# fusiyuan2010/CSC

Hardware: AMD Instinct MI355X
Metric: encode MB/s (10^6 input bytes / wall-clock) on enwik9 stand-in, -m3 -d64m; stream bit-exact vs reference (higher is better)
Workload: dtype u8/u32 (byte + 32-bit integer work; 12-bit probabilities, 64-bit range-coder low)

## Files before the change

csc_amd/csrc/csc_kernels_dp4.inc:

```

constexpr uint32_t kD4Rec = 256;
constexpr uint32_t kD4CandEnt = kD4Rec * 4;
constexpr uint32_t kD4RefEnt = 256;
constexpr uint32_t kD4Ent = kD4CandEnt + kD4RefEnt;
constexpr uint32_t kD4LA = 48;
constexpr uint32_t kD4Waves = 12;
DEV uint32_t d4_role(uint32_t w)
{
    constexpr uint32_t roles[12] = { 0, 6, 7, 1, 8, 5, 4, 2, 8, 8, 9, 3 };
    return w < 12 ? roles[w] : 8u;
}
constexpr uint32_t kD4Requested = 0xFFFFFFFFu;
#ifndef D4_IDLE_MUL
#define D4_IDLE_MUL 1
#endif
constexpr int kD4IdleSleep = 4 * D4_IDLE_MUL;
constexpr uint32_t kD4RefreshAt = 32;
constexpr uint32_t kD4MaxGood = 16;
constexpr uint32_t kD6Ring = 128;
constexpr uint32_t kD6MRing = 64;
constexpr uint32_t kD4MultiMax = 768;

struct Dp4X {
    uint32_t sb_seq, sb_ack, quit, abort;
// ... 1436 lines not shown
#ifdef CSCMI_TIMERS
                const uint32_t k_run0 = k;
#endif
                do {
#ifdef CSCMI_TIMERS_FINE
                    const unsigned long long tt0 = __builtin_readcyclecounter();
                    unsigned long long tt1 = 0;
#endif
                    pf_load();
                    d5_pad<D5_PAD_SPINE>();
                    const uint32_t st4 = (d5_bcast<D5F_BS>(LBL) >> 14) & 0xFCu;
                    const uint64_t tlr = *(volatile __attribute__((address_space(3))) uint64_t *)(b_tlr + (st4 << 4));
                    const uint32_t m32 = d5_bcast<D5F_M32>(LBL), tbu = d5_bcast<D5F_TBV>(LBL);
                    const uint32_t has1 = ((m32 & 3u) + 1u) >> 2;
                    const uint32_t p1f = tbu >> 16;
                    uint32_t E, cond0;
                    auto own = [&]() {
                        const uint32_t cl = tree + (tbu & 0xFFFFu);
                        const uint32_t k1m = (uint32_t)((int32_t)(p1f - cl) >> 31) & (0u - has1);
                        const uint32_t price = (p1f & k1m) | (cl & ~k1m);
                        const uint32_t eBS = k | (((st4 | (k1m & 2u)) & 0x3Fu) << 16);
                        const uint32_t tbE = ((uint32_t)(tlr >> 32) & k1m) | ((uint32_t)tlr & ~k1m);
                        E = (LBL >> shv) + ((price & mP) | c_left);
                        E = (eBS & mBS) | (E & ~mBS);
                        E = (k1m & 1u & mD) | (E & ~mD);
                        E = (tbE & mTBV) | (E & ~mTBV);
                        cond0 = (E & m_lsign) | ((v_lp - kD5Zone1) >> 31);
                    };
                    own();
                    const uint32_t want = winhi | k;
                    uint32_t late, wayout;
                    auto looks = [&]() {
                        late = (((uint32_t)prog - want) | ((uint32_t)(prog >> 32) - want)) >> 16;
                        const uint32_t g = (V.x ^ 1u) | (v_reach ^ j);
                        wayout = (V.w & D5V_OUT) | ((g - 1u) >> 31);
                    };
                    looks();
                    uint32_t LBLn, em;
                    auto merge = [&]() {
                        const uint32_t d = (T1 & mlow) - (T0 & mlow);
                        const uint32_t ds = (uint32_t)__builtin_amdgcn_mov_dpp((int)d, 0x55, 0xF, 0xF, false);
                        const uint32_t x = d != 0 ? d : ds;
                        const uint32_t t1 = d5_bcast<D5F_P>((uint32_t)((int32_t)x >> 31));
                        const uint32_t BEST = (T1 & t1) | (T0 & ~t1);
                        em = d5_bcast<D5F_P>((uint32_t)((int32_t)(E - BEST) >> 31));
                        LBLn = ((E & em) | (BEST & ~em)) | rfl;
                        asm volatile("" :: "v"(LBLn));
                    };
                    merge();
                    if (__builtin_expect(__ballot((late | wayout | cond0) != 0) != 0, 0)) {
                        if (__ballot(late != 0) != 0) {
                            uint32_t spins = 0;
                            for (;;) {
                                pf_load();
                                looks();
                                if (__ballot(late != 0) == 0) break;
                                if ((++spins & 0xFFFu) == 0 && (lds_vload(&X->abort) || spins > (kDpSpinLimit << 4))) {
                                    if (!lds_vload(&X->abort)) *(lds_vu32 *)&X->abort = 0x400D0000u | (k & 0xFFFFu);
                                    run = RUN_ABORT;
                                    break;
                                }
                            }
                            own();
                            merge();
#ifdef CSCMI_TIMERS_FINE
                            tt1 = __builtin_readcyclecounter();
#endif
                        }
                        if (run == RUN_ON && __ballot((wayout | cond0) != 0) != 0) {
                            const bool zone = __ballot(((v_lp - kD5Zone1) >> 31) != 0) != 0;
                            const bool out = __ballot(wayout != 0) != 0;
                            run = (zone || (out && D5DBG(8u))) ? RUN_GENERAL : out ? RUN_OUT : RUN_ASK;
                        }
                        if (run != RUN_ON) kstop = 0;
                    }
                    if (__builtin_expect(run == RUN_ON, 1)) {
                    LBL = LBLn;
                    *lds_at(st_a) = LBL;
                    k++;
                    *(lds_vu32 *)&X->lab_seq = k + 1u;
#ifdef CSCMI_TIMERS_FINE
                    if (tr_on && k <= 50) { unsigned long long *T = TR + (4 + k - 1) * 12; T[0] = tt0; T[1] = tt1; T[2] = __builtin_readcyclecounter(); T[8] = UNI(em) & 1u; }
#endif
                    st_a = (st_a & ~st_and) | ((st_a + st_inc) & st_and);
                    v_lp -= V.w & 0xFFFFu; v_reach = max(v_reach, j + V.x);
                    j = k - 1u;
                    pf_next();
                    }
                } while (k < kstop);
                vnext = j;
#ifdef CSCMI_TIMERS
                n_straight += k - k_run0;
#endif
                if (__builtin_expect(run != RUN_ON, 0)) {
                    const uint32_t wpos = sb0 + w0 + k;
                    if (run == RUN_ASK) {
                        const raw_vec4 e2 = *(lds_vvec4 *)&X->ent[(rdlane(LBL, D5F_I0) & 0xFFFFu) + vz];
                        uint32_t nm, nl;
                        mask_at(e2, wpos, nm, nl);
                        LBL = (nm & mM32) | (nl & c_left) | (LBL & ~(mM32 | c_left));
                        if (__ballot(nl == 0) == 0) continue;
#ifdef CSCMI_TIMERS
                        if (lane == 0) atomicAdd(&X->wtm[32], 1u);
#endif
                        leave = 1;
                    } else if (run == RUN_OUT) {
                        const uint32_t v0 = UNI(V.x), v1 = UNI(V.y), v2 = UNI(V.z), v3 = UNI(V.w);
                        v_lp -= v3 & 0xFFFFu;
                        if (j == 0 && (v3 & D5V_NONE)) { kind = DP_SEEN_EXIT; end = 0; }
                        else {
                            kind = (v0 == 1u) ? DP_EXIT_LIT : DP_EXIT_MATCH; end = j;
                            a0l = v0; a0code = v1; a0eid = v2 & 0xFFFFu; a0slot = v2 >> 16;
                        }
                        leave = 2;
                    } else if (run == RUN_ABORT) { err = 1; kind = DP_ABORT; leave = 2; }
                    else {
#ifdef CSCMI_TIMERS
                        if (lane == 0) atomicAdd(&X->wtm[35], 1u);
#endif
                        leave = 1;
                    }
                    break;
                }
            }
            vP = rdlane(LBL, D5F_P) | vz; vBS = rdlane(LBL, D5F_BS) | vz; vD = rdlane(LBL, D5F_D) | vz; vI0 = rdlane(LBL, D5F_I0) | vz; vI1 = rdlane(LBL, D5F_I1) | vz;
            if (leave == 2) break;
        }

        const uint32_t p = w0 + k, wpos = sb0 + p;
        *(lds_vu32 *)&X->m_pos = w0 + vnext; *(lds_vu32 *)&X->m_ids[0] = vI0; *(lds_vu32 *)&X->m_ids[1] = vI1;
        bool done = false;
        if (__builtin_expect(!done, 0)) {
#ifdef CSCMI_TIMERS
            const unsigned long long tg0 = __builtin_readcyclecounter();
            n_gen++;
#endif
            uint32_t cP = UNI(vP), cD = UNI(vD), cBS = UNI(vBS), cI0 = UNI(vI0), cI1 = UNI(vI1), lp_int = UNI(v_lp), reach = UNI(v_reach);
            const uint32_t state = (cBS >> 16) & 0x3Fu;
            bool out = false;
            uint32_t eP = kDpInf, eD = 0, eBS = 0;
            if (k < aplimit) {
                uint32_t rid_v = __builtin_amdgcn_perm(cI1, cI0, sel_rid);
                raw_vec4 en = *(lds_vvec4 *)&X->ent[rid_v];
                const uint32_t fwv = *(lds_vu32 *)&X->fwd[rid_v];
                const uint32_t tb = UNI(*(lds_vu32 *)&X->tab[state][8]);
                uint32_t tree = *(volatile __attribute__((address_space(3))) uint16_t *)&X->litp[lit_seq & 3u][p & (kD4Rec - 1)];
                {
                    const bool ask = (lane < 4) & (fwv == 0) & (wpos - en.y >= 64u) & (wpos - en.y < 0x80000000u);
                    if (__builtin_expect(__ballot(ask) != 0, 0)) rq_head = UNI(d4_ask(__ballot(ask), rid_v, wpos, rq_head));
                    const bool sw = (lane < 4) & (fwv != 0) & (fwv != kD4Requested);
                    if (__builtin_expect(__ballot(sw) != 0, 0)) {
                        lds_fence();
                        const uint32_t sm = 0u - (uint32_t)sw;
                        rid_v = ((fwv - 1u) & sm) | (rid_v & ~sm);
                        en = *(lds_vvec4 *)&X->ent[rid_v];
                        const uint32_t n0 = rdlane(rid_v, 0), n1 = rdlane(rid_v, 1), n2 = rdlane(rid_v, 2), n3 = rdlane(rid_v, 3);
                        cI0 = n0 | (n1 << 16); cI1 = n2 | (n3 << 16);
                    }
                }
                const uint32_t ex = UNI(en.x), ey = UNI(en.y), ez = UNI(en.z), ew = UNI(en.w);
                const uint32_t off = wpos - ey;
                const uint64_t m = (((uint64_t)ew << 32) | ez) >> (off & 63u);
                const uint32_t room = 64u - (off & 63u);
                uint32_t rl0 = umin((~m) ? (uint32_t)__builtin_ctzll(~m) : 64u, room);
                if (__builtin_expect(off >= 64u || rl0 >= room || (ey < ex && ex <= wpos), 0)) rl0 = UNI(d4_rep_direct(true, wpos, ex, size - p));
                const uint32_t has1 = rl0 >= 2u ? 1u : 0u;
                if (__builtin_expect(p >= lit_ok, 0)) {
                    lit_ok = UNI(d4_wait_lit(p, lit_seq & 0x3FFFFu));
                    if (!lit_ok) { err = 1; kind = DP_ABORT; out = true; }
                    tree = *(volatile __attribute__((address_space(3))) uint16_t *)&X->litp[lit_seq & 3u][p & (kD4Rec - 1)];
                }
                const uint32_t litf = tb & 0xFFFFu, p1f = tb >> 16;
                uint32_t c1 = UNI(tree) + litf, k1 = 0;
                if (has1 && p1f < c1) { c1 = p1f; k1 = 1; }
                eP = cP + c1; eD = k1; eBS = k | (((state * 4u + (k1 ? 2u : 0u)) & 0x3Fu) << 16);
            }
            if (__builtin_expect(lp_int < 192u && !have_new, 0)) { d6_wait_match_trees(); d4_len_price_rebuild(X->lenp_new); have_new = 1; }
            for (uint32_t pass = 0; pass < 2 && !out; pass++) {
                if (pass == 1 && !(lp_int < kD5Zone2 && k < aplimit)) break;
                const uint32_t vneed = k + pass;
                if (!d5_wait_edges(X, winhi, vneed, k, vz)) { err = 1; kind = DP_ABORT; out = true; break; }
                lds_fence();
                for (; vnext < vneed; vnext++) {
                    const uint32_t j = vnext;
                    const raw_vec4 V = *(lds_vvec4 *)&X->ver[j & 15u];
                    const uint32_t v0 = UNI(V.x), v1 = UNI(V.y), v2 = UNI(V.z), v3 = UNI(V.w);
                    const uint32_t nt = v3 & 0xFFFFu;
                    if (j == 0 && (v3 & D5V_NONE)) { kind = DP_SEEN_EXIT; end = 0; out = true; break; }
                    if (v3 & D5V_PRICED) {
                        if (lp_int < nt) { lp_int = 4096u - (nt - lp_int - 1u); refreshed = 1; }
                        else lp_int -= nt;
                    }
                    const bool exit_lit = v0 == 1 && reach == j;
                    const bool exit_match = v0 >= good || (v0 > 1 && v0 + j >= aplimit);
                    if (exit_lit || exit_match) {
                        kind = exit_lit ? DP_EXIT_LIT : DP_EXIT_MATCH; end = j;
                        a0l = v0; a0code = v1; a0eid = v2 & 0xFFFFu; a0slot = v2 >> 16;
                        out = true;
                        break;
                    }
                    reach = max(reach, j + v0);
                }
            }
            if (!out && k == aplimit) { kind = DP_EXIT_LIMIT; end = k; out = true; }
            if (!out) {
                const uint32_t t = k + 1u;
                uint32_t bP = kDpInf, bD = 0, bBS = 0, bI0 = 0, bI1 = 0;
                if (k >= 1) {
                    const raw_vec4 A = *(lds_vvec4 *)&X->tent[t & 1u][t & 15u][0];
                    bP = UNI(A.x); bBS = UNI(A.y); bD = UNI(A.z); bI0 = UNI(A.w); bI1 = UNI(*(lds_vu32 *)&X->tent[t & 1u][t & 15u][4]);
                }
                if (k >= 2) {
                    const raw_vec4 B = *(lds_vvec4 *)&X->tent[k & 1u][t & 15u][0];
                    const uint32_t qP = UNI(B.x), qBS = UNI(B.y), qD = UNI(B.z), qI0 = UNI(B.w), qI1 = UNI(*(lds_vu32 *)&X->tent[k & 1u][t & 15u][4]);
                    if (qP < bP || (qP == bP && (qBS & 0xFFFFu) < (bBS & 0xFFFFu))) { bP = qP; bD = qD; bBS = qBS; bI0 = qI0; bI1 = qI1; }
                }
                if (eP < bP) { bP = eP; bD = eD; bBS = eBS; bI0 = cI0; bI1 = cI1; }
                cP = bP; cD = bD; cBS = bBS; cI0 = bI0; cI1 = bI1;
                k++;
                raw_vec4 lb;
                lb.x = cP; lb.y = cBS | (refreshed << 31) | (lp_int < kD5Zone2 ? (lp_int + 1u) << 24 : 0u); lb.z = cI0; lb.w = cI1;
                *(lds_vvec4 *)&X->lab[k & 15u] = lb;
                L->fin2[k * 2u] = cD; L->fin2[k * 2u + 1u] = cBS;
#ifdef CSCMI_TIMERS
                if (k < 64) { X->dbgq[k][0] = cP; X->dbgq[k][5] = eP; X->dbgq[k][6] = 2; X->dbgq[k][7] = lp_int; }
#endif
                lds_fence();
                *(lds_vu32 *)&X->lab_seq = k + 1u;
            }
            vP = cP | vz; vD = cD | vz; vBS = cBS | vz; vI0 = cI0 | vz; vI1 = cI1 | vz; v_lp = lp_int | vz; v_reach = reach | vz;
            fI0 = cI0; fI1 = cI1;
            if (!out) pf_label();
#ifdef CSCMI_TIMERS
            t_gen += __builtin_readcyclecounter() - tg0;
#endif
            if (out) break;
        }
    }
#ifdef CSCMI_TIMERS
    const unsigned long long tse = __builtin_readcyclecounter();
    if (lane == 0) { atomicAdd(&X->wtm[13], (uint32_t)(tse - ts0) >> 4); atomicAdd(&X->wtm[14], n_straight); atomicAdd(&X->wtm[15], 1u);
        atomicAdd(&X->wtm[24], (uint32_t)(ts0 - tsp) >> 4); atomicAdd(&X->wtm[25], (uint32_t)t_first >> 4); atomicAdd(&X->wtm[26], (uint32_t)t_poll >> 4);
        atomicAdd(&X->wtm[27], (uint32_t)t_gen >> 4); atomicAdd(&X->wtm[28], n_gen); atomicAdd(&X->wtm[29], (uint32_t)(tse - t_last) >> 4); }
#endif
    lds_fence();
    *(lds_vu32 *)&X->lab_seq = kD5Stop;
    if (refreshed) { if (lane < 32) L->len_price[lane] = X->lenp_new[lane]; lds_fence(); }
    uint32_t f0 = kind == DP_EXIT_LIMIT ? fI0 : UNI(X->lab[end & 15u].z);
    uint32_t f1 = kind == DP_EXIT_LIMIT ? fI1 : UNI(X->lab[end & 15u].w);
    d5_forward_ids(X, lane, sel_rid, f0, f1);
    *(lds_vu32 *)&X->m_pos = w0 + end; *(lds_vu32 *)&X->m_ids[0] = f0; *(lds_vu32 *)&X->m_ids[1] = f1;
    {
        raw_vec4 o0, o1, o2;
        o0.x = kind; o0.y = end; o0.z = a0l; o0.w = a0code; o1.x = a0eid; o1.y = a0slot; o1.z = f0; o1.w = f1;
        o2.x = v_lp; o2.y = lit_seq; o2.z = rq_head; o2.w = err;
        *(lds_vvec4 *)&X->o_kind = o0; *(lds_vvec4 *)&X->o_a0eid = o1; *(lds_vvec4 *)&X->o_lp_int = o2;
    }
    lds_fence();
#ifdef CSCMI_TIMERS
    if (lane == 0) atomicAdd(&X->wtm[30], (uint32_t)(__builtin_readcyclecounter() - tse) >> 4);
#endif
}

DEV void d4_request(Sc &c, Dp4X *X, uint32_t id, uint32_t base, uint32_t &rq_head)
{
    if (rq_head - lds_vload(&X->rq_tail) >= 16u) return;
    X->rq[rq_head & 15u][0] = id;
    X->rq[rq_head & 15u][1] = base;
    X->fwd[id] = kD4Requested;
    rq_head++;
    lds_fence();
    lds_vstore(&X->rq_head, rq_head);
}

DEV bool d4_rebase_reps(Sc &c, Dp4X *X, uint32_t base, uint32_t &rq_head, bool wait)
{
    for (uint32_t r = 0; r < 4; r++) {
        const uint32_t id = lds_vload(&X->rid[r]);
        const uint32_t f = lds_vload(&X->fwd[id]);
        if (f == 0) {
            uint32_t spins = 0;
            while (rq_head - lds_vload(&X->rq_tail) >= 16u) if (!d4_spin(c, X, spins, 3)) return false;
            d4_request(c, X, id, base, rq_head);
        }
    }
    if (!wait) return true;
    for (uint32_t r = 0; r < 4; r++) {
        uint32_t id = lds_vload(&X->rid[r]);
        uint32_t spins = 0, f;
        while ((f = lds_vload(&X->fwd[id])) == kD4Requested) if (!d4_spin(c, X, spins, 4)) return false;
        if (f) { lds_fence(); X->rid[r] = f - 1; }
    }
    return true;
}


struct D6Cur { uint32_t lt_head, lt_seen, mt_head, mt_seen; };
DEV bool d6_join(Sc &c, Dp4X *X, D6Cur &q, bool lit_only = false);
DEV bool d6_room(Sc &c, Dp4X *X, uint32_t need, D6Cur &q)
{
    if (__builtin_expect(c.q_room < need, 0)) {
#ifdef CSCMI_TIMERS
        const uint64_t t0 = __builtin_readcyclecounter();
#endif
        if (!d6_join(c, X, q)) return false;
#ifdef CSCMI_TIMERS
        const uint64_t t1 = __builtin_readcyclecounter();
#endif
        q_publish(c);
        c.q_room = kCoderQ - 64u - q_wait_room(c, 64u + need);
#ifdef CSCMI_TIMERS
        if (c.lane == 0) { atomicAdd(&X->wtm[40], 1u); atomicAdd(&X->wtm[41], (uint32_t)(t1 - t0) >> 4); atomicAdd(&X->wtm[42], (uint32_t)(__builtin_readcyclecounter() - t1) >> 4); atomicAdd(&X->wtm[46], c.q_room >> 4); }
#endif
    }
    return true;
}
DEV bool d6_literal(Sc &c, Dp4X *X, uint32_t sym, D6Cur &q)
{
    if (__builtin_expect(q.lt_head - q.lt_seen >= kD6Ring - 8u, 0)) {
        uint32_t spins = 0;
        while (q.lt_head - (q.lt_seen = lds_vload(&X->lt_done)) >= kD6Ring - 8u) if (!d4_spin(c, X, spins, 12)) return false;
    }
    const uint32_t fidx = P_STATE + c.state * 3;
    const uint32_t pold = c.L->P[fidx];
    c.L->P[fidx] = p_update(0, pold);
    c.Q->e[c.q_head & (kCoderQ - 1)] = 0x80000000u | pold;
    *(lds_vu32 *)&X->lt_rec[q.lt_head & (kD6Ring - 1)] = c.ctx | (sym << 8) | (c.q_head << 16);
    q.lt_head++;
    *(lds_vu32 *)&X->lt_pub = q.lt_head;
    c.q_head += 9; c.q_room -= 9;
    c.state = (c.state * 4) & 0x3F;
    c.ctx = sym;
    c.st_lit++;
    return true;
}
DEV void d6_flags(Sc &c, uint32_t nf, uint32_t idx, uint32_t bit)
{
    const bool on = c.lane < nf;
    const uint32_t i = on ? idx : kPDumpE;
    const uint32_t p = c.L->P[i];
    c.L->P[i] = p + (uint32_t)((int32_t)((bit ? 0xFFFu : 31u) - p) >> 5);
    c.Q->e[(c.q_head + (on ? c.lane : 63u)) & (kCoderQ - 1)] = 0x80000000u | (bit << 12) | p;
    c.q_head += nf; c.q_room -= nf;
}
DEV uint32_t d6_len_slots(uint32_t len) { return len < 8 ? 4u : len < 16 ? 5u : 9u; }
DEV bool d6_tree_record(Sc &c, Dp4X *X, uint32_t w0, uint32_t w1, uint32_t nslots, D6Cur &q)
{
    if (__builtin_expect(q.mt_head - q.mt_seen >= kD6MRing, 0)) {
        uint32_t spins = 0;
        while (q.mt_head - (q.mt_seen = lds_vload(&X->mt_done)) >= kD6MRing) if (!d4_spin(c, X, spins, 14)) return false;
    }
    *(lds_vu32 *)&X->mt_rec[q.mt_head & (kD6MRing - 1)][0] = w0 | (c.q_head << 16);
    *(lds_vu32 *)&X->mt_rec[q.mt_head & (kD6MRing - 1)][1] = w1;
    q.mt_head++;
    *(lds_vu32 *)&X->mt_pub = q.mt_head;
    c.q_head += nslots; c.q_room -= nslots;
    return true;
}
DEV bool d6_match(Sc &c, Dp4X *X, uint32_t dist, uint32_t len, D6Cur &q)
{
    d6_flags(c, 2, P_STATE + c.state * 3 + c.lane, 1u);
    const uint32_t sbits = len == 0 ? 3u : len <= 2 ? 4u : 5u;
    const uint32_t slot = dist_slot(dist), extra_bits = slot > 2 ? slot - 2 : 0;
    const uint32_t ndir = extra_bits > 4 ? (extra_bits - 4 > 16 ? 2u : 1u) : 0u;
    if (!d6_tree_record(c, X, 0u | (len << 1), dist, d6_len_slots(len) + sbits + ndir + (extra_bits ? 4u : 0u), q)) return false;
    c.state = (c.state * 4 + 1) & 0x3F;
    c.st_match++;
    return true;
}
DEV bool d6_rep_match(Sc &c, Dp4X *X, uint32_t rep_idx, uint32_t len, D6Cur &q)
{
    const uint32_t s3 = c.state * 3, k = c.lane;
    const uint32_t idx = k < 3 ? P_STATE + s3 + k : P_REPDIST + s3 - 1u + (k == 3 ? 1u : 2u | (rep_idx >> 1));
    const uint32_t bit = k < 3 ? (0x5u >> k) & 1u : (rep_idx >> ((4u - k) & 1u)) & 1u;
    d6_flags(c, 5, idx, bit);
    if (!d6_tree_record(c, X, 1u | (len << 1), 0u, d6_len_slots(len), q)) return false;
    c.state = (c.state * 4 + 3) & 0x3F;
    c.st_match++;
    return true;
}
DEV void d6_rep0len1(Sc &c)
{
    d6_flags(c, 3, P_STATE + c.state * 3 + c.lane, c.lane == 0 ? 1u : 0u);
    c.ctx = 0;
    c.state = (c.state * 4 + 2) & 0x3F;
    c.st_match++;
}
DEV bool d6_encode_nonlit(Sc &c, Dp4X *X, uint32_t ulen, uint32_t udist, D6Cur &q)
{
    EncLds *L = c.L;
    if (udist <= 4) {
        if (ulen == 1 && udist == 1) d6_rep0len1(c);
        else {
            if (!d6_rep_match(c, X, udist - 1, ulen - 2, q)) return false;
            uint32_t d = UNI(L->rep[udist - 1]);
            for (uint32_t k = udist - 1; k > 0; k--) L->rep[k] = UNI(L->rep[k - 1]);
            L->rep[0] = d;
        }
    } else {
        if (!d6_match(c, X, udist - 5, ulen - 2, q)) return false;
        uint32_t r0 = UNI(L->rep[0]), r1 = UNI(L->rep[1]), r2 = UNI(L->rep[2]);
        L->rep[3] = r2; L->rep[2] = r1; L->rep[1] = r0; L->rep[0] = udist - 4;
    }
    return true;
}
DEV uint32_t d6_chunk_shape(uint32_t nd, uint32_t ql, bool on)
{
    const uint32_t len = ql & 0xFFFFu;
    const uint32_t kind = nd == 0 ? 0u : nd > 4 ? 1u : (nd == 1 && len == 1) ? 2u : 3u;
    const uint32_t l2 = len - 2u, dist = nd - 5u;
    const uint32_t sbits = l2 == 0 ? 3u : l2 <= 2 ? 4u : 5u;
    const uint32_t slot = dist_slot(dist), extra_bits = slot > 2 ? slot - 2 : 0;
    const uint32_t ndir = extra_bits > 4 ? (extra_bits - 4 > 16 ? 2u : 1u) : 0u;
    const uint32_t nf = kind == 0 ? 1u : kind == 1 ? 2u : kind == 2 ? 3u : 5u;
    const uint32_t tree = kind == 0 ? 8u : kind == 2 ? 0u : d6_len_slots(l2) + (kind == 1 ? sbits + ndir + (extra_bits ? 4u : 0u) : 0u);
    return on ? kind | (nf << 2) | ((nf + tree) << 8) : 0u;
}
DEV void d6_chunk_flag(bool act, uint32_t idx, uint32_t bit, uint32_t qslot, uint64_t same)
{
    const uint64_t am = __ballot(act);
    if (am == 0) return;
    const uint32_t lane = threadIdx.x & 63u;
    same &= am;
    const uint64_t below = same & ((1ull << lane) - 1ull), above = (same >> lane) >> 1;
    const uint32_t rank = (uint32_t)__builtin_popcountll(below);
    const uint32_t prev = below ? 63u - (uint32_t)__builtin_clzll(below) : lane;
    uint32_t pold = 0;
    if (act) pold = g_lds4.base.P[idx];
    uint32_t pnew = p_update(bit, pold);
    for (uint32_t d = 1; __ballot(act && rank >= d) != 0; d++) {
        const uint32_t v = (uint32_t)__builtin_amdgcn_ds_bpermute((int)(prev * 4u), (int)pnew);
        if (act && rank == d) { pold = v; pnew = p_update(bit, pold); }
    }
    if (act && above == 0) g_lds4.base.P[idx] = pnew;
    if (act) g_lds4.q.e[qslot & (kCoderQ - 1)] = 0x80000000u | (bit << 12) | pold;
}
__device__ __noinline__ uint32_t d6_chunk_lanes(uint32_t nd, uint32_t ql, uint32_t shape, uint32_t qpos, uint32_t n_, uint32_t state0_, uint32_t ctx0_, uint32_t lt_head_, uint32_t mt_head_)
{
    Dp4X *X = &g_lds4.x;
    const uint32_t lane = threadIdx.x & 63u;
    const uint32_t n = UNI(n_), state0 = UNI(state0_), ctx0 = UNI(ctx0_), lt_head = UNI(lt_head_), mt_head = UNI(mt_head_);
    const bool on = lane < n;
    const uint32_t kind = shape & 3u, nf = (shape >> 2) & 7u;
    const uint32_t len = ql & 0xFFFFu, last = ql >> 16;
    const uint64_t b0 = __ballot(on && (kind & 1u)), b1 = __ballot(on && (kind & 2u));
    const uint64_t h0 = (b0 << 3) | ((state0 & 1u) << 2) | (((state0 >> 2) & 1u) << 1) | ((state0 >> 4) & 1u);
    const uint64_t h1 = (b1 << 3) | (((state0 >> 1) & 1u) << 2) | (((state0 >> 3) & 1u) << 1) | ((state0 >> 5) & 1u);
    const uint32_t a = (uint32_t)(lane >= 3 ? b0 >> (lane - 3u) : h0 >> lane) & 7u, b = (uint32_t)(lane >= 3 ? b1 >> (lane - 3u) : h1 >> lane) & 7u;
    const uint32_t state = ((a >> 2) & 1u) | (((b >> 2) & 1u) << 1) | (((a >> 1) & 1u) << 2) | (((b >> 1) & 1u) << 3) | ((a & 1u) << 4) | ((b & 1u) << 5);
    const uint32_t before = (uint32_t)__shfl_up((int)last, 1);
    const uint32_t ctx = lane == 0 ? ctx0 : before;
    const bool is_lit = on && kind == 0, has_tree = on && (kind & 1u);
    const uint64_t lm = __ballot(is_lit), tm = __ballot(has_tree);
    if (is_lit) {
        const uint32_t r = __builtin_amdgcn_mbcnt_hi((uint32_t)(lm >> 32), __builtin_amdgcn_mbcnt_lo((uint32_t)lm, 0u));
        *(lds_vu32 *)&X->lt_rec[(lt_head + r) & (kD6Ring - 1)] = ctx | (last << 8) | (qpos << 16);
    }
    if (lm) lds_vstore(&X->lt_pub, lt_head + (uint32_t)__builtin_popcountll(lm));
    if (has_tree) {
        const uint32_t r = __builtin_amdgcn_mbcnt_hi((uint32_t)(tm >> 32), __builtin_amdgcn_mbcnt_lo((uint32_t)tm, 0u));
        *(lds_vu32 *)&X->mt_rec[(mt_head + r) & (kD6MRing - 1)][0] = (kind == 3 ? 1u : 0u) | ((len - 2u) << 1) | ((qpos + nf) << 16);
        *(lds_vu32 *)&X->mt_rec[(mt_head + r) & (kD6MRing - 1)][1] = kind == 1 ? nd - 5u : 0u;
    }
    if (tm) lds_vstore(&X->mt_pub, mt_head + (uint32_t)__builtin_popcountll(tm));
    uint64_t same = 0;
    for (uint64_t rem = __ballot(on); rem;) {
        const uint32_t sv = rdlane(state, (uint32_t)__builtin_ctzll(rem));
        const uint64_t mm = __ballot(on && state == sv);
        same = state == sv ? mm : same;
        rem &= ~mm;
    }
    const uint32_t s3 = state * 3u, rep_hi = ((nd - 1u) >> 1) & 1u;
    const bool is_rep = on && kind == 3;
    d6_chunk_flag(on, P_STATE + s3, kind != 0 ? 1u : 0u, qpos, same);
    d6_chunk_flag(on && kind != 0, P_STATE + s3 + 1u, kind == 1 ? 1u : 0u, qpos + 1u, same);
    d6_chunk_flag(on && kind >= 2, P_STATE + s3 + 2u, kind == 3 ? 1u : 0u, qpos + 2u, same);
    d6_chunk_flag(is_rep, P_REPDIST + s3, rep_hi, qpos + 3u, same);
    const uint64_t hi = __ballot(is_rep && rep_hi);
    d6_chunk_flag(is_rep, P_REPDIST + s3 + 1u + rep_hi, (nd - 1u) & 1u, qpos + 4u, same & (rep_hi ? hi : ~hi));
    return rdlane(((state * 4u + kind) & 0x3Fu) | (last << 8), n - 1u);
}
DEV bool d6_join(Sc &c, Dp4X *X, D6Cur &q, bool lit_only)
{
    uint32_t spins = 0;
    if (q.lt_seen != q.lt_head) {
        while ((q.lt_seen = lds_vload(&X->lt_done)) != q.lt_head) if (!d4_spin(c, X, spins, 13)) return false;
        dp_fence();
    }
    if (!lit_only && q.mt_seen != q.mt_head) {
        while ((q.mt_seen = lds_vload(&X->mt_done)) != q.mt_head) if (!d4_spin(c, X, spins, 15)) return false;
        lds_fence();
    }
    return true;
}
DEV void d6_trees(Sc &c)
{
    Dp4X *X = d4x(c);
    uint32_t done = 0, mdone = 0;
  for (;;) {
    uint32_t pub, mpub, idle = 0;
    for (;;) {
        pub = lds_vload(&X->lt_pub); mpub = lds_vload(&X->mt_pub);
        if (pub != done || mpub != mdone) break;
        if (lds_vload(&X->quit) || lds_vload(&X->abort)) return;
        if (idle < 48u) { idle++; __builtin_amdgcn_s_sleep(1 * D4_IDLE_MUL); }
        else __builtin_amdgcn_s_sleep(6 * D4_IDLE_MUL);
    }
    if (pub == done) {
        const uint32_t w0 = lds_vload(&X->mt_rec[mdone & (kD6MRing - 1)][0]), dist = lds_vload(&X->mt_rec[mdone & (kD6MRing - 1)][1]);
        const uint32_t len = (w0 >> 1) & 0xFFu, qpos = w0 >> 16;
        Decisions d; d.idx = 0; d.bit = 0; d.n = 0;
        dec_matchlen_1(c, d, len);
        uint32_t n_head = d.n, extra_bits = 0, extra_len = 0;
        if ((w0 & 1u) == 0) {
            uint32_t pdist_pos, sbits;
            if (len == 0) { pdist_pos = 0; sbits = 3; }
            else if (len <= 2) { pdist_pos = 16 * (len - 1) + 8; sbits = 4; }
            else if (len <= 5) { pdist_pos = 32 * (len - 3) + 8 + 16 * 2; sbits = 5; }
            else { pdist_pos = 32 * 3 + 8 + 16 * 2; sbits = 5; }
            const uint32_t slot = dist_slot(dist);
            extra_bits = slot > 2 ? slot - 2 : 0;
            dec_tree(c, d, P_DIST + pdist_pos, slot, sbits);
            n_head = d.n;
            if (extra_bits) {
                extra_len = dist - (1u << extra_bits) - 1;
                dec_tree(c, d, P_DIST_EXTRA + (extra_bits - 1) * 16, __brev(extra_len & 0x0Fu) >> 28, 4);
            }
        }
        const uint32_t pold = dec_apply(c, d);
        uint32_t ndir = 0;
        if (extra_bits > 4) {
            const uint32_t v = extra_len >> 4, l = extra_bits - 4;
            if (l <= 16) { g_lds4.q.e[(qpos + n_head) & (kCoderQ - 1)] = 0x40000000u | (l << 16) | (v & 0xFFFFu); ndir = 1; }
            else { g_lds4.q.e[(qpos + n_head) & (kCoderQ - 1)] = 0x40000000u | ((l - 16) << 16) | ((v >> 16) & 0xFFFFu);
                   g_lds4.q.e[(qpos + n_head + 1u) & (kCoderQ - 1)] = 0x40000000u | (16u << 16) | (v & 0xFFFFu); ndir = 2; }
        }
        {
            const uint32_t k = c.lane;
            const bool on = k < d.n;
            const uint32_t at = qpos + k + (k >= n_head ? ndir : 0u);
            lds_vu32 *const slot_p = on ? (lds_vu32 *)&g_lds4.q.e[at & (kCoderQ - 1)] : (lds_vu32 *)&g_lds4.q.pad;
            *slot_p = 0x80000000u | (d.bit << 12) | pold;
        }
        lds_fence();
        mdone++;
        lds_vstore(&X->mt_done, mdone);
    }
    while (done != pub) {
        const uint32_t nlit = umin(pub - done, 8u);
        const uint32_t lane = c.lane, i = lane >> 3, k = lane & 7u;
        const uint32_t rec = *(lds_vu32 *)&X->lt_rec[(done + i) & (kD6Ring - 1)];
        const uint32_t ctx = rec & 0xFFu, cc = ((rec >> 8) & 0xFFu) | 0x100u, qpos = rec >> 16;
        const uint32_t idx = cc >> (8u - k), bit = (cc >> (7u - k)) & 1u;
        const bool act = i < nlit;
        const uint32_t cell = act ? ctx * 256u + idx : 0x80000000u | lane;
        uint32_t pold = 0;
        if (act) pold = c.p_lit[cell];
        uint32_t prevj = 0;
        bool later = false;
#pragma unroll
        for (uint32_t j = 7; j >= 1; j--) {
            const uint32_t o = (uint32_t)__builtin_amdgcn_ds_bpermute((int)((lane - 8u * j) * 4u), (int)cell);
            prevj = (i >= j && o == cell) ? j : prevj;
            const uint32_t o2 = (uint32_t)__builtin_amdgcn_ds_bpermute((int)((lane + 8u * j) * 4u), (int)cell);
            later = later || (i + j < 8u && o2 == cell);
        }
        uint32_t pnew = p_update(bit, pold);
        const uint64_t cm = __ballot(prevj != 0);
        if (__builtin_expect(cm != 0, 0)) {
            for (uint32_t r = 1; r < nlit; r++) {
                if (((cm >> (8u * r)) & 0xFFull) == 0) continue;
                const uint32_t v = (uint32_t)__builtin_amdgcn_ds_bpermute((int)((lane - 8u * prevj) * 4u), (int)pnew);
                if (i == r && prevj != 0) { pold = v; pnew = p_update(bit, pold); }
            }
        }
        if (act && !later) c.p_lit[cell] = pnew;
        if (act) g_lds4.q.e[(qpos + 1u + k) & (kCoderQ - 1)] = 0x80000000u | (bit << 12) | pold;
        dp_fence();
        done += nlit;
        lds_vstore(&X->lt_done, done);
        pub = lds_vload(&X->lt_pub);
    }
  }
}

DEV void lz_compress_advanced_dp4(Sc &c, uint32_t size)
{
    EncLds *L = c.L;
    Dp4X *X = d4x(c);
    const uint32_t lane = c.lane;
    const uint32_t sb0 = c.wnd_curpos, pos0 = c.pos;
    uint32_t rq_head = lds_vload(&X->rq_head);
    uint32_t ev_seq = lds_vload(&X->ev_seq);
    bool ev_pending = false;
    {
        lds_vstore(&X->sb0, sb0); lds_vstore(&X->pos0, pos0); lds_vstore(&X->size, size);
        lds_vstore(&X->m_pos, 0);
        {
            const uint64_t wa = (uint64_t)(uintptr_t)c.wnd;
            X->io_wnd_lo = (uint32_t)wa; X->io_wnd_hi = (uint32_t)(wa >> 32); X->io_wnd_size = c.wnd_size; X->io_vld = c.vld_rge; X->io_good = c.lz_good_len;
            const uint64_t pa = (uint64_t)(uintptr_t)c.p_lit;
            X->io_plit_lo = (uint32_t)pa; X->io_plit_hi = (uint32_t)(pa >> 32);
        }
        dp_fence();
        const uint32_t seq = lds_vload(&X->sb_seq) + 1;
        lds_vstore(&X->sb_seq, seq);
        uint32_t spins = 0;
        while (lds_vload(&X->sb_ack) != seq) if (!d4_spin(c, X, spins, 5)) return;
        lds_fence();
        uint32_t id0 = 0;
        if (lane == 0) id0 = atomicAdd(&X->ref_head, 4u);
        id0 = UNI(id0);
        if (lane < 4) {
            const uint32_t nid = kD4CandEnt + ((id0 + lane) & (kD4RefEnt - 1));
            raw_vec4 en;
            en.x = L->rep[lane]; en.y = sb0 - 64u; en.z = 0; en.w = 0;
            X->ent[nid] = en;
            X->fwd[nid] = 0;
            X->rid[lane] = nid;
        }
        lds_fence();
        if (!d4_rebase_reps(c, X, sb0, rq_head, true)) return;
    }
    uint32_t gen = lds_vload(&X->gen);
    uint32_t lit_seq = lds_vload(&X->lit_req);
    D6Cur tq;
    tq.lt_head = lds_vload(&X->lt_pub); tq.lt_seen = lds_vload(&X->lt_done); tq.mt_head = lds_vload(&X->mt_pub); tq.mt_seen = lds_vload(&X->mt_done);

    for (uint32_t i = 0; i < size;) {
        if (lds_vload(&X->abort)) { c.error = lds_vload(&X->abort); return; }
        TM_DECL;
        const uint32_t w0 = i;
        lds_vstore(&X->m_pos, i);
        if (ev_pending) {
            uint32_t spins = 0;
            while (lds_vload(&X->ev_ack) != ev_seq) if (!d4_spin(c, X, spins, 6)) return;
            lds_fence();
            gen = lds_vload(&X->gen);
            ev_pending = false;
        }
        TM_ADD(c, 0);
        {
            const uint32_t rs = w0 & (kD4Rec - 1);
            const uint32_t tg = *(lds_vu32 *)&X->rec_tag[rs], hs = *(lds_vu32 *)&X->rec_hsum[rs];
            const uint32_t rid_l = *(lds_vu32 *)&X->rid[lane & 3u];
            const raw_vec4 en = *(lds_vvec4 *)&X->ent[rid_l];
            const uint32_t wpos = sb0 + w0, off = wpos - en.y;
            const uint32_t mlow = (uint32_t)((((uint64_t)en.w << 32) | en.z) >> (off & 63u));
            const uint32_t bad = (off >> 6) | ((((off & 63u) + 1u) >> 6) & mlow) | ((umin(en.x - en.y - 1u, 0x7FFFFFFFu) - off) >> 31) | (((mlow & 3u) + 1u) >> 2);
            if (UNI(tg) == d4_tag(gen, w0) && (UNI(hs) & 0xFFu) == 0 && __ballot(bad != 0) == 0 && w0 + 1u < size && !D5FLAG(30)) {
                if (!d6_room(c, X, 16u, tq)) return;
                if (!d6_literal(c, X, stage_byte(c, sb0 + w0), tq)) return;
                TM_ADD(c, 4);
                c.st_find++;
                i++;
                continue;
            }
        }
        if (!d6_join(c, X, tq, true)) return;
        TM_ADD(c, 5);
        if (__builtin_expect(c.error != 0, 0)) { if (!lds_vload(&X->abort)) lds_vstore(&X->abort, c.error); return; }
        X->io_w0 = w0; X->io_gen = gen; X->io_state0 = c.state; X->io_lp_int = c.lp_rebuild_int; X->io_lit_seq = lit_seq; X->io_rq_head = rq_head;
        lds_fence();
#ifdef CSCMI_TIMERS
        if (D5DBG(32u) && c.lane < 32) X->dbgl[c.lane] = L->len_price[c.lane];
#endif
#ifdef CSCMI_TIMERS
        const bool d5_here = (lds_vload(&X->dbg) >> 8) == 0 || D5DBG(64u) || pos0 + w0 < (lds_vload(&X->dbg) >> 8) * 16u;
#else
        const bool d5_here = true;
#endif
#ifdef CSCMI_TIMERS
        if (kD5Split && !D5DBG(16u) && d5_here) d5_spine();
        else d4_window();
#else
        (void)d5_here;
        d5_spine();
#endif
#ifdef CSCMI_TIMERS
        if (D5DBG(128u) && pos0 + w0 + 1024u >= (lds_vload(&X->dbg) >> 8) * 16u) { for (int q = 0; q < 100; q++) __builtin_amdgcn_s_sleep(127); }
#endif
#ifdef CSCMI_TIMERS
        if (D5DBG(32u) && lds_vload(&X->o_end) < 150u && c.S->stats.trace[62][0] == 0
            && (!D5DBG(64u) || (pos0 + w0 < (lds_vload(&X->dbg) >> 8) * 16u && pos0 + w0 + 16u >= (lds_vload(&X->dbg) >> 8) * 16u))) {
            auto sig = [&]() -> uint32_t {
                uint32_t h = lds_vload(&X->o_kind) * 0x9E3779B1u + lds_vload(&X->o_end);
                h = h * 0x85EBCA6Bu + lds_vload(&X->o_a0l); h = h * 0x85EBCA6Bu + lds_vload(&X->o_a0code); h = h * 0x85EBCA6Bu + lds_vload(&X->o_lp_int);
                if (lds_vload(&X->o_kind) == DP_EXIT_MATCH) { h = h * 0x85EBCA6Bu + lds_vload(&X->o_a0slot); if (lds_vload(&X->o_a0code) > 4) h = h * 0x85EBCA6Bu + UNI(X->ent[lds_vload(&X->o_a0eid)].x); }
                { const uint32_t f0 = lds_vload(&X->o_fin_i0), f1 = lds_vload(&X->o_fin_i1);
                  h = h * 31u + UNI(X->ent[f0 & 0xFFFFu].x); h = h * 31u + UNI(X->ent[f0 >> 16].x); h = h * 31u + UNI(X->ent[f1 & 0xFFFFu].x); h = h * 31u + UNI(X->ent[f1 >> 16].x); }
                for (uint32_t t = lds_vload(&X->o_end); t;) {
                    const uint32_t b = UNI(L->fin2[t * 2u + 1u] & 0xFFFFu), d = UNI(L->fin2[t * 2u]);
                    h = (h ^ (t * 31u + d)) * 0x01000193u;
                    t = b;
                }
                return h;
            };
            auto sig2 = [&]() -> uint32_t {
                uint32_t h = 0;
                for (uint32_t q = 0; q < 32; q++) h = h * 31u + UNI(L->len_price[q]);
                return h;
            };
            auto snap = [&](unsigned long long *T) {
                uint32_t hf = 0, he = 0;
                for (uint32_t q = c.lane; q < kD4Ent; q += 64) { hf += X->fwd[q] * (q * 2u + 1u); const raw_vec4 e = X->ent[q]; he += (e.x * 3u + e.y * 5u + e.z * 7u + e.w * 11u) * (q * 2u + 1u); }
                for (int o = 32; o; o >>= 1) { hf += __shfl_xor(hf, o); he += __shfl_xor(he, o); }
                if (c.lane == 0) {
                    T[0] = hf; T[1] = he; T[2] = lds_vload(&X->ref_head); T[3] = lds_vload(&X->rq_head) | ((unsigned long long)lds_vload(&X->rq_tail) << 32);
                    T[4] = lds_vload(&X->lit_req) | ((unsigned long long)lds_vload(&X->lit_done) << 32); T[5] = lds_vload(&X->m_pos);
                    T[6] = lds_vload(&X->m_ids[0]) | ((unsigned long long)lds_vload(&X->m_ids[1]) << 32); T[7] = lds_vload(&X->gen) | ((unsigned long long)lds_vload(&X->ins_head) << 32);
                    T[8] = lds_vload(&X->o_fin_i0) | ((unsigned long long)lds_vload(&X->o_fin_i1) << 32); T[9] = lds_vload(&X->o_kind) | ((unsigned long long)lds_vload(&X->o_end) << 32);
                    T[10] = lds_vload(&X->o_a0eid) | ((unsigned long long)lds_vload(&X->o_a0slot) << 32); T[11] = pos0 + w0;
                }
            };
            if (D5DBG(64u)) snap(c.S->stats.trace[58]);
            const uint32_t t5 = sig2();
            const uint32_t s5 = sig(), k5 = lds_vload(&X->o_kind), e5 = lds_vload(&X->o_end), l5 = lds_vload(&X->o_lp_int), a5 = lds_vload(&X->o_a0l), c5 = lds_vload(&X->o_a0code);
            const uint32_t g0 = lds_vload(&X->o_fin_i0), g1 = lds_vload(&X->o_fin_i1);
            const uint32_t r5a = UNI(X->ent[g0 & 0xFFFFu].x), r5b = UNI(X->ent[g0 >> 16].x), r5c = UNI(X->ent[g1 & 0xFFFFu].x), r5d = UNI(X->ent[g1 >> 16].x), sl5 = lds_vload(&X->o_a0slot);
            if (c.lane < 60) { c.S->stats.trace[c.lane][0] = L->fin2[c.lane * 2u]; c.S->stats.trace[c.lane][1] = L->fin2[c.lane * 2u + 1u] & 0xFFFFu; }
            X->io_lit_seq = lds_vload(&X->o_lit_seq);
            if (c.lane < 32) L->len_price[c.lane] = X->dbgl[c.lane];
            lds_fence();
            d4_window();
            const uint32_t s4 = sig();
            if (D5DBG(64u)) snap(c.S->stats.trace[59]);
            const uint32_t t4 = sig2();
            if (t4 != t5 && c.S->stats.trace[62][0] == 0 && c.lane == 0) { unsigned long long *T = c.S->stats.trace[62]; T[0] = 2; T[1] = pos0 + w0; T[2] = t5; T[3] = t4; T[4] = lds_vload(&X->io_lp_int); T[5] = lds_vload(&X->o_lp_int); T[6] = lds_vload(&X->o_end); }
            if (s4 != s5 && c.S->stats.trace[62][0] == 0) {
                if (c.lane < 60) { c.S->stats.trace[c.lane][2] = L->fin2[c.lane * 2u]; c.S->stats.trace[c.lane][3] = L->fin2[c.lane * 2u + 1u] & 0xFFFFu; c.S->stats.trace[c.lane][4] = X->dbgp[c.lane]; for (int q = 0; q < 7; q++) c.S->stats.trace[c.lane][5 + q] = X->dbgq[c.lane][q == 6 ? 7 : q]; c.S->stats.trace[c.lane][11] |= (unsigned long long)X->dbgq[c.lane][6] << 32; }
                if (c.lane == 0) {
                    unsigned long long *T = c.S->stats.trace[62];
                    T[0] = 1; T[1] = pos0 + w0; T[2] = k5; T[3] = e5; T[4] = l5; T[5] = a5; T[6] = c5;
                    T[7] = lds_vload(&X->o_kind); T[8] = lds_vload(&X->o_end); T[9] = lds_vload(&X->o_lp_int); T[10] = lds_vload(&X->o_a0l); T[11] = lds_vload(&X->io_lp_int);
                    unsigned long long *U = c.S->stats.trace[63];
                    const uint32_t q0 = lds_vload(&X->o_fin_i0), q1 = lds_vload(&X->o_fin_i1);
                    U[1] = r5a; U[2] = r5b; U[3] = r5c; U[4] = r5d; U[5] = sl5; U[6] = X->ent[q0 & 0xFFFFu].x; U[7] = X->ent[q0 >> 16].x; U[8] = X->ent[q1 & 0xFFFFu].x; U[9] = X->ent[q1 >> 16].x; U[10] = lds_vload(&X->o_a0slot);
                }
            }
        }
#endif
        const raw_vec4 o0 = *(lds_vvec4 *)&X->o_kind, o1 = *(lds_vvec4 *)&X->o_a0eid, o2 = *(lds_vvec4 *)&X->o_lp_int;
        const uint32_t kind = UNI(o0.x), end = UNI(o0.y);
        uint32_t a0l = UNI(o0.z);
        const uint32_t a0code = UNI(o0.w), a0eid = UNI(o1.x), a0slot = UNI(o1.y);
        const uint32_t fin_i0 = UNI(o1.z), fin_i1 = UNI(o1.w);
        c.lp_rebuild_int = UNI(o2.x); lit_seq = UNI(o2.y); rq_head = UNI(o2.z);
        c.st_find += end + (kind == DP_EXIT_LIMIT ? 0u : 1u);
        TM_ADD(c, 1);
#ifdef CSCMI_TIMERS
        if (D5FLAG(29) && c.S->stats.trace[62][0] == 0) {
            const uint32_t thr = lds_vload(&X->tr_win) & 0x1FFFFFFFu;
            if (sb0 + w0 <= thr && thr < sb0 + w0 + end + 1u + (kind == DP_EXIT_MATCH ? a0l : 0u)) {
                if (c.lane < 60) { c.S->stats.trace[c.lane][0] = L->fin2[c.lane * 2u]; c.S->stats.trace[c.lane][1] = L->fin2[c.lane * 2u + 1u]; }
                if (c.lane == 0) {
                    unsigned long long *T = c.S->stats.trace[62];
                    T[0] = 7; T[1] = sb0 + w0; T[2] = kind; T[3] = end; T[4] = a0l; T[5] = a0code; T[6] = a0slot; T[7] = X->ent[fin_i0 & 0xFFFFu].x; T[8] = X->ent[fin_i0 >> 16].x;
                    T[9] = X->ent[fin_i1 & 0xFFFFu].x; T[10] = X->ent[fin_i1 >> 16].x; T[11] = c.state;
                    unsigned long long *U = c.S->stats.trace[63];
                    U[1] = L->rep[0]; U[2] = L->rep[1]; U[3] = L->rep[2]; U[4] = L->rep[3]; U[5] = fin_i0; U[6] = fin_i1; U[7] = X->rid[0] | ((unsigned long long)X->rid[1] << 32); U[8] = X->rid[2] | ((unsigned long long)X->rid[3] << 32);
                    U[9] = X->fwd[X->rid[0]]; U[10] = X->ent[X->rid[0]].y; U[11] = lds_vload(&X->rq_head) | ((unsigned long long)lds_vload(&X->rq_tail) << 32);
                }
            }
        }
#endif
        if (kind == DP_ABORT || UNI(o2.w)) { c.error = lds_vload(&X->abort) | 0x08000000u; return; }
        if (kind == DP_SEEN_EXIT) {
            if (lane < 4) X->rid[lane] = lane == 0 ? fin_i0 & 0xFFFFu : lane == 1 ? fin_i0 >> 16 : lane == 2 ? fin_i1 & 0xFFFFu : fin_i1 >> 16;
            wave_fence();
            if (!d6_room(c, X, 16u, tq)) return;
            if (!d6_literal(c, X, stage_byte(c, sb0 + w0), tq)) return;
            i++;
            TM_ADD(c, 7);
            continue;
        }
        c.wnd_curpos = sb0 + w0 + end;
        if (kind == DP_EXIT_MATCH) {
            if (a0l >= 64u && a0slot >= 4) {
                const uint32_t mp = sb0 + w0 + end, d = a0code - 4u;
                const bool fwd = a0slot == 4 ? (mp > d) : (mp >= d);
                const uint32_t cp = fwd ? mp - d : mp + c.wnd_size - d;
                a0l = wave_prefix_from(c, mp, cp, 64u, umin(size - (w0 + end), c.wnd_size - cp));
            }
            lds_vstore(&X->ev_s, w0 + end); lds_vstore(&X->ev_len, a0l);
            lds_fence();
            ev_seq++;
            lds_vstore(&X->ev_seq, ev_seq);
            ev_pending = true;
        }
        {
            const uint32_t id = lane == 0 ? fin_i0 & 0xFFFFu : lane == 1 ? fin_i0 >> 16 : lane == 2 ? fin_i1 & 0xFFFFu : fin_i1 >> 16;
            if (lane < 4) { X->rid[lane] = id; L->rep[lane] = X->ent[id].x; }
        }
        wave_fence();
        if (kind == DP_EXIT_MATCH) {
            const uint32_t i0 = lds_vload(&X->rid[0]), i1 = lds_vload(&X->rid[1]), i2 = lds_vload(&X->rid[2]), i3 = lds_vload(&X->rid[3]);
            if (a0code > 4) { X->rid[0] = a0eid; X->rid[1] = i0; X->rid[2] = i1; X->rid[3] = i2; }
            else if (a0code == 2) { X->rid[0] = i1; X->rid[1] = i0; }
            else if (a0code == 3) { X->rid[0] = i2; X->rid[1] = i0; X->rid[2] = i1; }
            else if (a0code == 4) { X->rid[0] = i3; X->rid[1] = i0; X->rid[2] = i1; X->rid[3] = i2; }
            wave_fence();
            if (a0l > kD4RefreshAt && w0 + end + a0l < size && !d4_rebase_reps(c, X, sb0 + w0 + end + a0l, rq_head, false)) return;
        }
        TM_ADD(c, 6);
        uint32_t pm_lo = 0, pm_hi = 0;
        for (uint32_t t = end; t;) {
            const uint32_t ch = t >> 6;
            const uint32_t Bv = L->fin2[(ch * 64u + lane) * 2u + 1u] & 0xFFFFu;
            uint64_t m = 0;
            do { m |= 1ull << (t & 63u); t = rdlane(Bv, t & 63u); } while (t && (t >> 6) == ch);
            pm_lo = d4_m0_wrlane(pm_lo, UNI((uint32_t)m), UNI(ch));
            pm_hi = d4_m0_wrlane(pm_hi, UNI((uint32_t)(m >> 32)), UNI(ch));
        }
        TM_ADD(c, 2);
        for (uint32_t ch = 0; ch <= (end >> 6); ch++) {
            const uint64_t m = ((uint64_t)rdlane(pm_hi, ch) << 32) | rdlane(pm_lo, ch);
            if (m == 0) continue;
            const uint32_t n = (uint32_t)__builtin_popcountll(m);
            const uint32_t q = ch * 64u + lane;
            const uint32_t back = L->fin2[q * 2u + 1u] & 0xFFFFu, ndv = L->fin2[q * 2u];
            const uint32_t sidx = w0 + q + 15u;
            const uint32_t lastb = (L->stage[sidx >> 2] >> ((sidx & 3u) * 8u)) & 0xFFu;
            const bool isp = (m >> lane) & 1ull;
            const uint32_t rank = __builtin_amdgcn_mbcnt_hi((uint32_t)(m >> 32), __builtin_amdgcn_mbcnt_lo((uint32_t)m, 0u));
            const uint32_t tgt = (isp ? rank : n + (lane - rank)) * 4u;
            const uint32_t d_nd = (uint32_t)__builtin_amdgcn_ds_permute((int)tgt, (int)ndv);
            const uint32_t d_ql = (uint32_t)__builtin_amdgcn_ds_permute((int)tgt, (int)((q - back) | (lastb << 16)));
            const uint32_t shape = d6_chunk_shape(d_nd, d_ql, lane < n);
            uint32_t qoff = 0, need = 0;
#pragma unroll
            for (uint32_t b = 0; b < 5; b++) {
                const uint64_t pm = __ballot((shape >> (8u + b)) & 1u);
                qoff += __builtin_amdgcn_mbcnt_hi((uint32_t)(pm >> 32), __builtin_amdgcn_mbcnt_lo((uint32_t)pm, 0u)) << b;
                need += (uint32_t)__builtin_popcountll(pm) << b;
            }
            const uint32_t nl = (uint32_t)__builtin_popcountll(__ballot(lane < n && (shape & 3u) == 0)), nm = (uint32_t)__builtin_popcountll(__ballot(shape & 1u));
            if (!d6_room(c, X, need, tq)) return;
            if (tq.lt_head + nl - tq.lt_seen > kD6Ring - 8u) tq.lt_seen = lds_vload(&X->lt_done);
            if (tq.mt_head + nm - tq.mt_seen > kD6MRing) tq.mt_seen = lds_vload(&X->mt_done);
            const bool at_once = c.q_room >= need && tq.lt_head + nl - tq.lt_seen <= kD6Ring - 8u && tq.mt_head + nm - tq.mt_seen <= kD6MRing;
            TM_ADD(c, 3);
            if (at_once) {
                const uint32_t sc = UNI(d6_chunk_lanes(d_nd, d_ql, shape, c.q_head + qoff, n, c.state, c.ctx, tq.lt_head, tq.mt_head));
                c.state = sc & 0x3Fu; c.ctx = sc >> 8;
                c.q_head += need; c.q_room -= need;
                tq.lt_head += nl; tq.mt_head += nm;
                c.st_lit += nl; c.st_match += n - nl;
                continue;
            }
            for (uint32_t r = 0; r < n; r++) {
                const uint32_t nd = rdlane(d_nd, r), ql = rdlane(d_ql, r);
                const uint32_t len = ql & 0xFFFFu, last = ql >> 16;
                if (nd == 0) {
                    if (!d6_literal(c, X, last, tq)) return;
                    TMF_ADD(c, 4);
                } else if (nd <= 4) {
                    if (len == 1 && nd == 1) d6_rep0len1(c);
                    else if (!d6_rep_match(c, X, nd - 1, len - 2, tq)) return;
                    c.ctx = last;
                    TMF_ADD(c, 7);
                } else {
                    if (!d6_match(c, X, nd - 5, len - 2, tq)) return;
                    c.ctx = last;
                    TMF_ADD(c, 7);
                }
            }
        }
        i += end;
        if (!d6_room(c, X, 256u, tq)) return;
        if (kind == DP_EXIT_LIT) {
            if (!d6_literal(c, X, stage_byte(c, sb0 + i), tq)) return;
            i++;
        } else if (kind == DP_EXIT_MATCH) {
            if (a0l >= 145u) {
                if (!d6_join(c, X, tq)) return;
                lz_encode_nonlit(c, a0l, a0code);
            } else if (!d6_encode_nonlit(c, X, a0l, a0code, tq)) return;
            c.st_slide += a0l - 1;
            i += a0l;
            c.ctx = stage_byte(c, sb0 + i - 1);
// ... 178 lines not shown
```

Before: 2.739.

## Process up to sixteen literals per batch in the literal-modeling wave

```diff
diff --git a/csc_amd/csrc/csc_kernels_dp4.inc b/csc_amd/csrc/csc_kernels_dp4.inc
--- a/csc_amd/csrc/csc_kernels_dp4.inc
+++ b/csc_amd/csrc/csc_kernels_dp4.inc
@@ -1762,6 +1762,7 @@
     if (__builtin_expect(c.q_room < need, 0)) {
 #ifdef CSCMI_TIMERS
         const uint64_t t0 = __builtin_readcyclecounter();
+        const uint32_t out0 = (q.lt_head - lds_vload(&X->lt_done)) + (q.mt_head - lds_vload(&X->mt_done));
 #endif
         if (!d6_join(c, X, q)) return false;
 #ifdef CSCMI_TIMERS
@@ -1770,7 +1771,8 @@
         q_publish(c);
         c.q_room = kCoderQ - 64u - q_wait_room(c, 64u + need);
 #ifdef CSCMI_TIMERS
-        if (c.lane == 0) { atomicAdd(&X->wtm[40], 1u); atomicAdd(&X->wtm[41], (uint32_t)(t1 - t0) >> 4); atomicAdd(&X->wtm[42], (uint32_t)(__builtin_readcyclecounter() - t1) >> 4); atomicAdd(&X->wtm[46], c.q_room >> 4); }
+        if (c.lane == 0) { atomicAdd(&X->wtm[40], 1u); atomicAdd(&X->wtm[41], (uint32_t)(t1 - t0) >> 4); atomicAdd(&X->wtm[42], (uint32_t)(__builtin_readcyclecounter() - t1) >> 4); atomicAdd(&X->wtm[46], c.q_room >> 4);
+                           atomicAdd(&X->wtm[31], out0); if (t1 - t0 < 2048u) atomicAdd(&X->wtm[47], 1u); }
 #endif
     }
     return true;
@@ -2007,35 +2009,72 @@
         lds_vstore(&X->mt_done, mdone);
     }
     while (done != pub) {
-        const uint32_t nlit = umin(pub - done, 8u);
+        const uint32_t nlit = umin(pub - done, 16u), n_a = umin(nlit, 8u), n_b = nlit - n_a;
         const uint32_t lane = c.lane, i = lane >> 3, k = lane & 7u;
-        const uint32_t rec = *(lds_vu32 *)&X->lt_rec[(done + i) & (kD6Ring - 1)];
-        const uint32_t ctx = rec & 0xFFu, cc = ((rec >> 8) & 0xFFu) | 0x100u, qpos = rec >> 16;
-        const uint32_t idx = cc >> (8u - k), bit = (cc >> (7u - k)) & 1u;
-        const bool act = i < nlit;
-        const uint32_t cell = act ? ctx * 256u + idx : 0x80000000u | lane;
-        uint32_t pold = 0;
-        if (act) pold = c.p_lit[cell];
-        uint32_t prevj = 0;
-        bool later = false;
+        const uint32_t rec_a = *(lds_vu32 *)&X->lt_rec[(done + i) & (kD6Ring - 1)], rec_b = *(lds_vu32 *)&X->lt_rec[(done + 8u + i) & (kD6Ring - 1)];
+        const uint32_t cc_a = ((rec_a >> 8) & 0xFFu) | 0x100u, cc_b = ((rec_b >> 8) & 0xFFu) | 0x100u;
+        const uint32_t bit_a = (cc_a >> (7u - k)) & 1u, bit_b = (cc_b >> (7u - k)) & 1u;
+        const bool act_a = i < n_a, act_b = i < n_b;
+        const uint32_t cell_a = act_a ? (rec_a & 0xFFu) * 256u + (cc_a >> (8u - k)) : 0x80000000u | lane;
+        const uint32_t cell_b = act_b ? (rec_b & 0xFFu) * 256u + (cc_b >> (8u - k)) : 0x80000040u | lane;
+        uint32_t pold_a = 0, pold_b = 0;
+        if (act_a) pold_a = c.p_lit[cell_a];
+        if (act_b) pold_b = c.p_lit[cell_b];
+        uint32_t prev_a = 0, prev_b = 0;
+        bool later_a = false, later_b = false;
 #pragma unroll
         for (uint32_t j = 7; j >= 1; j--) {
-            const uint32_t o = (uint32_t)__builtin_amdgcn_ds_bpermute((int)((lane - 8u * j) * 4u), (int)cell);
-            prevj = (i >= j && o == cell) ? j : prevj;
-            const uint32_t o2 = (uint32_t)__builtin_amdgcn_ds_bpermute((int)((lane + 8u * j) * 4u), (int)cell);
-            later = later || (i + j < 8u && o2 == cell);
-        }
-        uint32_t pnew = p_update(bit, pold);
-        const uint64_t cm = __ballot(prevj != 0);
-        if (__builtin_expect(cm != 0, 0)) {
-            for (uint32_t r = 1; r < nlit; r++) {
-                if (((cm >> (8u * r)) & 0xFFull) == 0) continue;
-                const uint32_t v = (uint32_t)__builtin_amdgcn_ds_bpermute((int)((lane - 8u * prevj) * 4u), (int)pnew);
-                if (i == r && prevj != 0) { pold = v; pnew = p_update(bit, pold); }
-            }
-        }
-        if (act && !later) c.p_lit[cell] = pnew;
-        if (act) g_lds4.q.e[(qpos + 1u + k) & (kCoderQ - 1)] = 0x80000000u | (bit << 12) | pold;
+            const uint32_t o = (uint32_t)__builtin_amdgcn_ds_bpermute((int)((lane - 8u * j) * 4u), (int)cell_a);
+            prev_a = (i >= j && o == cell_a) ? j : prev_a;
+            const uint32_t o2 = (uint32_t)__builtin_amdgcn_ds_bpermute((int)((lane + 8u * j) * 4u), (int)cell_a);
+            later_a = later_a || (i + j < 8u && o2 == cell_a);
+        }
+        uint32_t from_a = 0;
+        if (n_b) {
+#pragma unroll
+            for (uint32_t j = 7; j >= 1; j--) {
+                const uint32_t o = (uint32_t)__builtin_amdgcn_ds_bpermute((int)((lane - 8u * j) * 4u), (int)cell_b);
+                prev_b = (i >= j && o == cell_b) ? j : prev_b;
+                const uint32_t o2 = (uint32_t)__builtin_amdgcn_ds_bpermute((int)((lane + 8u * j) * 4u), (int)cell_b);
+                later_b = later_b || (i + j < 8u && o2 == cell_b);
+            }
+#pragma unroll
+            for (uint32_t j = 0; j < 8; j++) {
+                const uint32_t r = (i + j) & 7u;
+                const uint32_t oa = (uint32_t)__builtin_amdgcn_ds_bpermute((int)((lane + 8u * j) * 4u), (int)cell_a);
+                from_a = (oa == cell_b && r + 1u > from_a) ? r + 1u : from_a;
+                const uint32_t ob = (uint32_t)__builtin_amdgcn_ds_bpermute((int)((lane + 8u * j) * 4u), (int)cell_b);
+                later_a = later_a || ob == cell_a;
+            }
+        }
+        uint32_t pnew_a = p_update(bit_a, pold_a);
+        const uint64_t cm_a = __ballot(prev_a != 0);
+        if (__builtin_expect(cm_a != 0, 0)) {
+            for (uint32_t r = 1; r < n_a; r++) {
+                if (((cm_a >> (8u * r)) & 0xFFull) == 0) continue;
+                const uint32_t v = (uint32_t)__builtin_amdgcn_ds_bpermute((int)((lane - 8u * prev_a) * 4u), (int)pnew_a);
+                if (i == r && prev_a != 0) { pold_a = v; pnew_a = p_update(bit_a, pold_a); }
+            }
+        }
+        if (n_b) {
+            if (__ballot(from_a != 0)) {
+                const uint32_t v = (uint32_t)__builtin_amdgcn_ds_bpermute((int)(((from_a - 1u) * 8u + k) * 4u), (int)pnew_a);
+                pold_b = from_a ? v : pold_b;
+            }
+            uint32_t pnew_b = p_update(bit_b, pold_b);
+            const uint64_t cm_b = __ballot(prev_b != 0);
+            if (__builtin_expect(cm_b != 0, 0)) {
+                for (uint32_t r = 1; r < n_b; r++) {
+                    if (((cm_b >> (8u * r)) & 0xFFull) == 0) continue;
+                    const uint32_t v = (uint32_t)__builtin_amdgcn_ds_bpermute((int)((lane - 8u * prev_b) * 4u), (int)pnew_b);
+                    if (i == r && prev_b != 0) { pold_b = v; pnew_b = p_update(bit_b, pold_b); }
+                }
+            }
+            if (act_b && !later_b) c.p_lit[cell_b] = pnew_b;
+            if (act_b) g_lds4.q.e[((rec_b >> 16) + 1u + k) & (kCoderQ - 1)] = 0x80000000u | (bit_b << 12) | pold_b;
+        }
+        if (act_a && !later_a) c.p_lit[cell_a] = pnew_a;
+        if (act_a) g_lds4.q.e[((rec_a >> 16) + 1u + k) & (kCoderQ - 1)] = 0x80000000u | (bit_a << 12) | pold_a;
         dp_fence();
         done += nlit;
         lds_vstore(&X->lt_done, done);
```

Result: faster. 2.825 (median of 6 runs) (+3.1%).
